# SpectacularAI/HybVIO

Hardware: NVIDIA H100
Metric: stereo frames/sec (752x480, 150 tracks) (higher is better)
Workload: dtype u8/s16 fixed-point + f32 (pyramid, LK), f64 (EKF)

## Files before the change

hybvio_b200/csrc/ekf.cuh:

```cuda
#pragma once
#include <cuda_runtime.h>

#define EKF_POS 0
#define EKF_VEL 3
#define EKF_ORI 6
#define EKF_BGA 10
#define EKF_BAA 13
#define EKF_BAT 16
#define EKF_SFT 19
#define EKF_CAM 20
#define EKF_INER 20
#define EKF_POSE 7
#define EKF_MAP_POINT 3
#define EKF_Q_ACC 0
#define EKF_Q_GYRO 3
#define EKF_Q_BGA_DRIFT 6
#define EKF_Q_BAA_DRIFT 9
#define EKF_Q_DIM 12

#define EKF_NT 512
#define EKF_SMALL_MAXN 8
#define EKF_SMALL_MAXL 32

struct EkfBufs {
    double* m;
    double* P;
    double* P2;
    double* work;
    double* cwork;
    double* Hs;
    double* Q;
    double* dydx;
    double* res;
    int N;
    int trail;
    int mapDim;
};

#define EKF_MODE_CHECK 0
#define EKF_MODE_UPDATE 1
#define EKF_MODE_CHECK_UPDATE 2

#define EKF_OP_DENSE 0
#define EKF_OP_ZUPT 1
#define EKF_OP_ZRUPT 2
#define EKF_OP_PSEUDO_VELOCITY 3
#define EKF_OP_POSITION 4
#define EKF_OP_ZERO_HEIGHT 5
#define EKF_OP_ORIENTATION 6
#define EKF_OP_AUGMENT 7

struct EkfUpdateArgs {
    EkfBufs b;
    const double* H;
    const double* f;
    const double* y;
    double ysmall[EKF_SMALL_MAXN];
    int n, l;
    int op;
    int mode;
    double Rdiag;
    double noiseScale;
    double rmseThr;
    double chi2Thr;
    int skipChi2;
    int normalizeAll;
    int symmetrize;
    int dropIdx;
    double augNoisePos, augNoiseOri;
    double defaultSpeed;
    int useGlobalWork;
    int symFirst;
    double* sig;
    double sigSeq;
    const int* gateI; int gateIExpect;
    const double* gateD; double gateDExpect;
    const int* counter; int counterMax;
    int* bump;
    double* slot;
    int lateH;
    int rowChunk;
    double* specP; double* specM;
    double Rdiag2;
};

__device__ __forceinline__ void ekf_report(const EkfUpdateArgs& a, double st, double chi2, double flag)
{
    a.b.res[0] = st; a.b.res[1] = chi2; a.b.res[2] = flag;
    if (a.slot) { a.slot[0] = st; a.slot[1] = chi2; a.slot[2] = flag; }
    if (a.sig) {
        a.sig[0] = st; a.sig[1] = chi2; a.sig[2] = flag;
        __threadfence_system();
        ((volatile double*)a.sig)[3] = a.sigSeq;
    }
}

#define EKF_MAX_BATCH 24
#define EKF_RES_STRIDE 32
struct EkfCheckItem {
    const double* H; const double* f; const double* y;
    int n, l;
    double Rdiag, chi2Thr, rmseThr;
    int skipChi2, pad;
};
struct EkfCheckBatch { int count; int pad; EkfCheckItem it[EKF_MAX_BATCH]; };

#define EKF_MAX_PREDICT 16
struct EkfPredictSample {
    double dt;
    double xg[3], xa[3];
    double baaDecay, bgaDecay;
    double qBaa, qBga;
    int normAfter, pad;
};
struct EkfPredictArgs {
    EkfBufs b;
    double gravity;
    double* meanOut;
    int count;
    EkfPredictSample s[EKF_MAX_PREDICT];
};

#define EKF_EW_SYMMETRIZE 1
#define EKF_EW_UNAUGMENT 2
#define EKF_EW_NORMALIZE 3
#define EKF_EW_TRANSLATE 4
#define EKF_EW_TRANSFORM 5
#define EKF_EW_INSERT_MAP_POINT 6
#define EKF_EW_LOCK_BIASES 7
#define EKF_EW_CONDITION_LAST_POSE 8
#define EKF_EW_INIT_ORIENTATION 9
struct EkfEwArgs {
    EkfBufs b;
    int op;
    int ival0;
    double dval[8];
};

cudaError_t ekf_launch_update(const EkfUpdateArgs& a, cudaStream_t s);
bool ekf_cluster2_fits(int n, int l, int N, bool joseph);
int ekf_cluster2_chunk_rows(int n, int l, int N);
cudaError_t ekf_launch_update_cluster2(const EkfUpdateArgs& a, cudaStream_t s);
cudaError_t ekf_launch_check_batch2(const EkfUpdateArgs& a, const EkfCheckBatch& b, cudaStream_t s, const EkfUpdateArgs* aug = nullptr);
cudaError_t ekf_launch_group_cluster2(const EkfUpdateArgs* hArgs, const EkfUpdateArgs* dArgs, int count, cudaStream_t s);
cudaError_t ekf_launch_group_predict(const EkfPredictArgs* hArgs, const EkfPredictArgs* dArgs, int count, cudaStream_t s);
struct TmArgs;
cudaError_t ekf_launch_predict(const EkfPredictArgs& a, cudaStream_t s);
cudaError_t ekf_launch_elementwise(const EkfEwArgs& a, cudaStream_t s);
```

hybvio_b200/csrc/ekf_cluster2.cu:

```cuda
#include <cooperative_groups.h>
#include "hv_device_once.cuh"
#include <math.h>
#include <stdlib.h>
namespace cg = cooperative_groups;

#ifdef HV_EKF_TIMING
#define EK2_PHASE(i) do { if (c == 0 && tid == 0) { unsigned long long t_; asm volatile("mov.u64 %0, %%globaltimer;" : "=l"(t_)); a.b.res[8 + (i)] = (double)t_; } } while (0)
#endif
#include "ekf_cluster2.cuh"

__global__ void __launch_bounds__(EK2_NT) ekf_update_cluster2_kernel(EkfUpdateArgs a)
{
    extern __shared__ __align__(16) double ek2_sm[];
    ek2_body<false>(a, ek2_sm, cg::this_cluster());
}

__global__ void __launch_bounds__(EK2_NT) ekf_update_cluster2_chunked_kernel(EkfUpdateArgs a)
{
    extern __shared__ __align__(16) double ek2_sm[];
    ek2_body<true>(a, ek2_sm, cg::this_cluster());
}

__global__ void __launch_bounds__(EK2_NT) ekf_check_batch_cluster2_kernel(EkfUpdateArgs a, EkfCheckBatch b, EkfUpdateArgs aug)
{
    extern __shared__ __align__(16) double ek2_sm[];
    cg::cluster_group cluster = cg::this_cluster();
    const int inst = blockIdx.x / EK2_C;
    if (inst >= b.count) a = aug;
    else {
        const EkfCheckItem& it = b.it[inst];
        a.H = it.H; a.f = it.f; a.y = it.y; a.n = it.n; a.l = it.l;
        a.Rdiag = it.Rdiag; a.chi2Thr = it.chi2Thr; a.rmseThr = it.rmseThr; a.skipChi2 = it.skipChi2;
        if (a.sig) a.sig += 4 * inst;
        if (a.slot) a.slot += 4 * inst;
    }
    a.b.res += (size_t)EKF_RES_STRIDE * inst;
    a.b.cwork += (size_t)inst * 10 * a.b.N * a.b.N;
    ek2_body<false>(a, ek2_sm, cluster);
}

__global__ void __launch_bounds__(EK2_NT) ekf_group_cluster2_kernel(const EkfUpdateArgs* __restrict__ args)
{
    extern __shared__ __align__(16) double ek2_sm[];
    ek2_group_body(args, blockIdx.x / EK2_C, ek2_sm, cg::this_cluster());
}

#define EK2_STATIC_SMEM (sizeof(double) * (2 + EK2_LINV_DOUBLES + 2 + EK2_MAXN) + 256)
#define EK2_SMEM_LIMIT (227 * 1024)

bool ekf_cluster2_fits(int n, int l, int N, bool joseph)
{
    return N <= EK2_MAXN && ek2_smem_bytes(n, l, N, joseph) + EK2_STATIC_SMEM <= EK2_SMEM_LIMIT;
}

int ekf_cluster2_chunk_rows(int n, int l, int N)
{
    if (N > EK2_MAXN) return 0;
    for (int h = n; h >= 1 && h >= (n < EK2_MIN_CHUNK ? n : EK2_MIN_CHUNK); h--)
        if (ek2_smem_bytes_chunked(h, n, l, N) + EK2_STATIC_SMEM <= EK2_SMEM_LIMIT) return h;
    return 0;
}

template <class K, class... Args>
static cudaError_t ek2_launch(K kernel, int nclusters, size_t smem, cudaStream_t s, Args... args)
{
    cudaLaunchConfig_t cfg = {};
    cfg.gridDim = dim3(EK2_C * nclusters); cfg.blockDim = dim3(EK2_NT); cfg.dynamicSmemBytes = smem; cfg.stream = s;
    cudaLaunchAttribute at[2];
    at[0].id = cudaLaunchAttributeClusterDimension; at[0].val.clusterDim.x = EK2_C; at[0].val.clusterDim.y = 1; at[0].val.clusterDim.z = 1;
    static const bool pdl = getenv("HV_EKF_NO_PDL") == nullptr;
    at[1].id = cudaLaunchAttributeProgrammaticStreamSerialization; at[1].val.programmaticStreamSerializationAllowed = 1;
    cfg.attrs = at; cfg.numAttrs = pdl ? 2 : 1;
    return cudaLaunchKernelEx(&cfg, kernel, args...);
}

template <class K>
static cudaError_t ek2_prepare(K kernel)
{
    return cudaFuncSetAttribute(kernel, cudaFuncAttributeMaxDynamicSharedMemorySize, (int)(EK2_SMEM_LIMIT - EK2_STATIC_SMEM));
}

cudaError_t ekf_launch_update_cluster2(const EkfUpdateArgs& a, cudaStream_t s)
{
    static bool seen[64], seenChunked[64];
    if (a.rowChunk > 0) {
        if (hv_first_use_on_device(seenChunked)) { cudaError_t e = ek2_prepare(ekf_update_cluster2_chunked_kernel); if (e != cudaSuccess) return e; }
        const size_t smem = ek2_smem_bytes_chunked(a.rowChunk < a.n ? a.rowChunk : a.n, a.n, a.l, a.b.N);
        return ek2_launch(ekf_update_cluster2_chunked_kernel, 1, smem, s, a);
    }
    if (hv_first_use_on_device(seen)) { cudaError_t e = ek2_prepare(ekf_update_cluster2_kernel); if (e != cudaSuccess) return e; }
    const size_t smem = ek2_smem_bytes(a.n, a.l, a.b.N, a.op == EKF_OP_AUGMENT);
    return ek2_launch(ekf_update_cluster2_kernel, 1, smem, s, a);
}

cudaError_t ekf_launch_check_batch2(const EkfUpdateArgs& a, const EkfCheckBatch& b, cudaStream_t s, const EkfUpdateArgs* aug)
{
    static bool seen[64];
    if (hv_first_use_on_device(seen)) { cudaError_t e = ek2_prepare(ekf_check_batch_cluster2_kernel); if (e != cudaSuccess) return e; }
    size_t smem = 0;
    for (int i = 0; i < b.count; i++) { const size_t v = ek2_smem_bytes(b.it[i].n, b.it[i].l, a.b.N, false); if (v > smem) smem = v; }
    if (aug) { const size_t v = ek2_smem_bytes(aug->n, aug->l, a.b.N, true); if (v > smem) smem = v; }
    return ek2_launch(ekf_check_batch_cluster2_kernel, b.count + (aug ? 1 : 0), smem, s, a, b, aug ? *aug : a);
}

cudaError_t ekf_launch_group_cluster2(const EkfUpdateArgs* hArgs, const EkfUpdateArgs* dArgs, int count, cudaStream_t s)
{
    static bool seen[64];
    if (hv_first_use_on_device(seen)) { cudaError_t e = ek2_prepare(ekf_group_cluster2_kernel); if (e != cudaSuccess) return e; }
    size_t smem = 0;
    for (int i = 0; i < count; i++) { const size_t v = ek2_smem_bytes(hArgs[i].n, hArgs[i].l, hArgs[i].b.N, hArgs[i].op == EKF_OP_AUGMENT); if (v > smem) smem = v; }
    return ek2_launch(ekf_group_cluster2_kernel, count, smem, s, dArgs);
}
```

hybvio_b200/csrc/ekf_cluster2.cuh:

```cuda
#pragma once
#include "ekf.cuh"
#include "hv_dmma.cuh"

#define EK2_NT 512
#define EK2_C 8
#define EK2_MAXN 768
#ifndef EK2_PHASE
#define EK2_PHASE(i) do { } while (0)
#endif
#ifndef EK2_ELIM_MARK
#define EK2_ELIM_MARK(i) do { } while (0)
#define EK2_ELIM_DECL
#endif

struct Ek2Geom { int B, X, W, T, PB, RS, EXTRA, SYM, oneStage, LD; };
__host__ __device__ inline int ek2_pad4mod16(int w) { return w + ((20 - (w & 15)) & 15); }
__host__ __device__ inline Ek2Geom ek2_geom(int n, int l, int N, bool joseph)
{
    Ek2Geom g;
    g.B = (N + EK2_C - 1) / EK2_C;
    g.LD = N + (((20 - (N & 15)) & 15) ? ((20 - (N & 15)) & 15) : 16);
    g.X = n * (l > g.LD ? l : g.LD);
    g.W = ek2_pad4mod16(n + g.B + 1 + (joseph ? n : 0));
    g.T = (n * g.W + 1) & ~1;
    g.PB = g.LD * g.B;
    const int MTn = (n + 7) >> 3;
    const int E = (64 * (MTn * (MTn + 1) / 2) + EK2_C - 1) / EK2_C;
    g.oneStage = n * n <= 1024 ? 1 : 0;
    g.RS = g.oneStage ? n * n : E;
    g.EXTRA = joseph ? N * EKF_POSE + 2 * 21 * g.LD + N * g.B : 0;
    g.SYM = n <= 8 ? N * g.B : 0;
    return g;
}
__host__ __device__ inline size_t ek2_smem_bytes(int n, int l, int N, bool joseph)
{
    const Ek2Geom g = ek2_geom(n, l, N, joseph);
    return ((size_t)g.X + g.T + g.PB + g.RS + g.EXTRA + g.SYM) * sizeof(double);
}
#define EK2_MIN_CHUNK 8
__host__ __device__ inline Ek2Geom ek2_geom_chunked(int h, int n, int l, int N)
{
    Ek2Geom g = ek2_geom(h, l, N, false);
    g.SYM = 0;
    g.EXTRA = (N + n + 1) & ~1;
    return g;
}
__host__ __device__ inline size_t ek2_smem_bytes_chunked(int h, int n, int l, int N)
{
    const Ek2Geom g = ek2_geom_chunked(h, n, l, N);
    return ((size_t)g.X + g.T + g.PB + g.RS + g.EXTRA) * sizeof(double);
}

__device__ __forceinline__ void ek2_copy8(double* __restrict__ dst, const double* __restrict__ src, int count, int tid)
{
    for (int base = 0; base < count; base += 8 * EK2_NT) {
        double r[8];
#pragma unroll
        for (int u = 0; u < 8; u++) { const int i = base + u * EK2_NT + tid; r[u] = i < count ? src[i] : 0.0; }
#pragma unroll
        for (int u = 0; u < 8; u++) { const int i = base + u * EK2_NT + tid; if (i < count) dst[i] = r[u]; }
    }
}
__device__ __forceinline__ void ek2_normalize_quat(double* q)
{
    const double z = (q[0] * q[0] + q[2] * q[2]) + (q[1] * q[1] + q[3] * q[3]);
    if (z > 0.0) { const double nrm = sqrt(z); q[0] /= nrm; q[1] /= nrm; q[2] /= nrm; q[3] /= nrm; }
}
__device__ __forceinline__ int ek2_aug_src(int i, int drop)
{
    if (i < EKF_CAM) return i;
    if (i < EKF_CAM + EKF_POSE) return -1;
    if (i < EKF_CAM + (drop + 1) * EKF_POSE) return i - EKF_POSE;
    return i;
}
__device__ __forceinline__ int ek2_special_col(int c) { return c < 3 ? EKF_POS + c : c < 7 ? EKF_ORI + c - 3 : EKF_CAM + c - 7; }

#define EK2_NI 4
__host__ __device__ inline void ek2_upper_tile(int tu, int& mt, int& nt)
{
    nt = (int)((sqrtf(8.0f * (float)tu + 1.0f) - 1.0f) * 0.5f);
    while ((nt + 1) * (nt + 2) / 2 <= tu) nt++;
    while (nt * (nt + 1) / 2 > tu) nt--;
    mt = tu - nt * (nt + 1) / 2;
}
template <int NI, bool UPPER, class FCI, class FST>
__device__ __forceinline__ void ek2_dmma_chunk(int M, int Nn, int K, int MT, int base, int stride, int lane, const double* A, int sAm, int sAk,
                                               const double* B, int sBk, int sBn, FCI cinit, FST store)
{
    const int g8 = lane >> 2, t4 = lane & 3;
    const int KF = K >> 2, tail = K & 3;
    const int dA = 4 * sAk, dB = 4 * sBk;
    double c0[NI], c1[NI];
    int row[NI], col[NI];
    const double* pa[NI]; const double* pb[NI];
#pragma unroll
    for (int q = 0; q < NI; q++) {
        const int tl = base + q * stride;
        int mt, nt;
        if (UPPER) ek2_upper_tile(tl, mt, nt); else { mt = tl % MT; nt = tl / MT; }
        row[q] = mt * 8 + g8; col[q] = nt * 8 + 2 * t4;
        const int rowc = min(row[q], M - 1), colbc = min(nt * 8 + g8, Nn - 1);
        pa[q] = A + (size_t)rowc * sAm + (size_t)t4 * sAk;
        pb[q] = B + (size_t)t4 * sBk + (size_t)colbc * sBn;
        c0[q] = cinit(rowc, min(col[q], Nn - 1)); c1[q] = cinit(rowc, min(col[q] + 1, Nn - 1));
    }
    int kt = 0;
    for (; kt + 2 <= KF; kt += 2) {
        double a0[NI], b0[NI], a1[NI], b1[NI];
#pragma unroll
        for (int q = 0; q < NI; q++) { a0[q] = pa[q][0]; b0[q] = pb[q][0]; a1[q] = pa[q][dA]; b1[q] = pb[q][dB]; pa[q] += 2 * dA; pb[q] += 2 * dB; }
#pragma unroll
        for (int q = 0; q < NI; q++) hv_dmma(c0[q], c1[q], a0[q], b0[q]);
#pragma unroll
        for (int q = 0; q < NI; q++) hv_dmma(c0[q], c1[q], a1[q], b1[q]);
    }
    if (kt < KF) {
        double a0[NI], b0[NI];
#pragma unroll
        for (int q = 0; q < NI; q++) { a0[q] = pa[q][0]; b0[q] = pb[q][0]; pa[q] += dA; pb[q] += dB; }
#pragma unroll
        for (int q = 0; q < NI; q++) hv_dmma(c0[q], c1[q], a0[q], b0[q]);
    }
    if (tail) {
        const bool kv = t4 < tail;
        double a0[NI], b0[NI];
#pragma unroll
        for (int q = 0; q < NI; q++) {
            const double xa = kv ? pa[q][0] : pa[q][-(ptrdiff_t)t4 * sAk];
            a0[q] = kv ? xa : 0.0;
            b0[q] = kv ? pb[q][0] : pb[q][-(ptrdiff_t)t4 * sBk];
        }
#pragma unroll
        for (int q = 0; q < NI; q++) hv_dmma(c0[q], c1[q], a0[q], b0[q]);
    }
    __syncwarp();
#pragma unroll
    for (int q = 0; q < NI; q++)
        if (row[q] < M && col[q] < Nn) store(row[q], col[q], c0[q], c1[q]);
}

template <bool UPPER = false, class FCI, class FST>
__device__ __forceinline__ void ek2_dmma_gemm(int M, int Nn, int K, int wrp, int lane, const double* A, int sAm, int sAk,
                                              const double* B, int sBk, int sBn, FCI cinit, FST store)
{
    const int MT = (M + 7) >> 3, NT = (Nn + 7) >> 3, tiles = UPPER ? MT * (MT + 1) / 2 : MT * NT;
    const int nwarps = EK2_NT / 32;
    if (M <= 0 || Nn <= 0) return;
    for (int base = wrp; base < tiles; base += nwarps * EK2_NI) {
        const int cnt = min(EK2_NI, (tiles - base + nwarps - 1) / nwarps);
        switch (cnt) {
            case 1: ek2_dmma_chunk<1, UPPER>(M, Nn, K, MT, base, nwarps, lane, A, sAm, sAk, B, sBk, sBn, cinit, store); break;
            case 2: ek2_dmma_chunk<2, UPPER>(M, Nn, K, MT, base, nwarps, lane, A, sAm, sAk, B, sBk, sBn, cinit, store); break;
            case 3: ek2_dmma_chunk<3, UPPER>(M, Nn, K, MT, base, nwarps, lane, A, sAm, sAk, B, sBk, sBn, cinit, store); break;
            default: ek2_dmma_chunk<4, UPPER>(M, Nn, K, MT, base, nwarps, lane, A, sAm, sAk, B, sBk, sBn, cinit, store); break;
        }
    }
}

#ifdef EK2_ELIM_OVERRIDE
#include EK2_ELIM_OVERRIDE
#else
#define EK2_LINV_DOUBLES 128
#define EK2_EB 8
__device__ __forceinline__ double ek2_rcp(double x)
{
#ifdef HV_EMU
    return 1.0 / x;
#else
    double r;
    asm("rcp.approx.ftz.f64 %0, %1;" : "=d"(r) : "d"(x));
    r = fma(fma(-x, r, 1.0), r, r);
    r = fma(fma(-x, r, 1.0), r, r);
    return r;
#endif
}

__device__ __forceinline__ void ek2_diag_factor(const double* T, int W, int r0, int nb, int lane, double* linv, volatile int* s_bad)
{
    double v[8];
    const int cidx = lane & 7;
#pragma unroll
    for (int i = 0; i < 8; i++) {
        const double t = T[(size_t)(r0 + min(i, nb - 1)) * W + r0 + min(cidx, nb - 1)];
        double x = (i == cidx) ? 1.0 : 0.0;
        if (lane < 8 && i < nb && cidx < nb) x = t;
        if (lane >= 16) x = 0.0;
        v[i] = x;
    }
    bool ok = true;
#pragma unroll
    for (int k = 0; k < 8; k++) {
        const double akk = __shfl_sync(0xffffffffu, v[k], k);
        double raw[8];
#pragma unroll
        for (int i = k + 1; i < 8; i++) raw[i] = __shfl_sync(0xffffffffu, v[k], i);
        if (!(akk > 0.0)) ok = false;
        const double r = rsqrt(akk);
        const double u = v[k] * r;
        v[k] = u;
#pragma unroll
        for (int i = k + 1; i < 8; i++) v[i] = fma(-(raw[i] * r), u, v[i]);
    }
    if (lane >= 8 && lane < 16) {
#pragma unroll
        for (int i = 0; i < 8; i++) linv[i * 8 + (lane - 8)] = v[i];
    }
    if (!ok && lane == 0) *s_bad = 1;
}

__device__ __forceinline__ bool ek2_block_eliminate(double* T, int W, int n, int ncols, int wrp, int lane, double* s_linv, volatile int* s_bad)
{
    const int g8 = lane >> 2, t4 = lane & 3;
    const int nwarps = EK2_NT / 32;
    const int MT = (n + 7) >> 3, CT = (ncols + 7) >> 3;
    EK2_ELIM_DECL
    if (wrp == 0) {
        if (lane == 0) *s_bad = 0;
        __syncwarp();
        ek2_diag_factor(T, W, 0, min(8, n), lane, s_linv, s_bad);
    }
    __syncthreads();
    for (int j = 0; j < MT; j++) {
        if (*s_bad) return false;
        const int r0 = 8 * j, nb = min(8, n - r0);
        const double* linv = s_linv + (j & 1) * 64;
        EK2_ELIM_MARK(0);
        for (int ct = j + wrp; ct < CT; ct += nwarps) {
            double c0 = 0.0, c1 = 0.0;
            const int colbc = min(8 * ct + g8, ncols - 1);
            double bf[2];
#pragma unroll
            for (int kt = 0; kt < 2; kt++) {
                const int k = kt * 4 + t4;
                const double x = T[(size_t)(r0 + min(k, nb - 1)) * W + colbc];
                bf[kt] = k < nb ? x : 0.0;
            }
#pragma unroll
            for (int kt = 0; kt < 2; kt++) hv_dmma(c0, c1, linv[g8 * 8 + kt * 4 + t4], bf[kt]);
            const int col = 8 * ct + 2 * t4;
            __syncwarp();
            if (g8 < nb) { if (col < ncols) T[(size_t)(r0 + g8) * W + col] = c0; if (col + 1 < ncols) T[(size_t)(r0 + g8) * W + col + 1] = c1; }
        }
        EK2_ELIM_MARK(1);
        __syncthreads();
        EK2_ELIM_MARK(2);
        if (j + 1 < MT) {
            const int first = j + 1;
            int total = 0;
            for (int mt = first; mt < MT; mt++) total += CT - mt;
            const bool ahead = wrp == 0;
            const int nwork = nwarps - nwarps / 4, widx = wrp - wrp / 4 - 1;
            const bool worker = (wrp & 3) != 0;
            const int rest = total - 1;
            int lo = ahead ? 0 : worker ? 1 + (int)(((long long)rest * widx) / nwork) : 0;
            const int hi = ahead ? 1 : worker ? 1 + (int)(((long long)rest * (widx + 1)) / nwork) : 0;
            const double* rowk0 = T + (size_t)(r0 + min(t4, nb - 1)) * W;
            const double* rowk1 = T + (size_t)(r0 + min(4 + t4, nb - 1)) * W;
            const bool k0v = t4 < nb, k1v = 4 + t4 < nb;
            if (ahead) {
                const int cb = 8 * first, am = min(cb + g8, ncols - 1);
                const double x0 = rowk0[am], x1 = rowk1[am];
                const int rowi = cb + g8, coli = cb + 2 * t4;
                double* crow = T + (size_t)min(rowi, n - 1) * W;
                double c0 = crow[min(coli, ncols - 1)], c1 = crow[min(coli + 1, ncols - 1)];
                hv_dmma(c0, c1, k0v ? -x0 : 0.0, x0);
                hv_dmma(c0, c1, k1v ? -x1 : 0.0, x1);
                __syncwarp();
                if (rowi < n) { if (coli < ncols) crow[coli] = c0; if (coli + 1 < ncols) crow[coli + 1] = c1; }
            } else if (worker) {
                int mt = first, nt, idx = min(lo, total - 1);
                while (idx >= CT - mt) { idx -= CT - mt; mt++; }
                nt = mt + idx;
                int curMt = -1;
                double a0 = 0.0, a1 = 0.0;
                for (; lo < hi; lo++) {
                    if (mt != curMt) {
                        const int am = min(8 * mt + g8, ncols - 1);
                        const double x0 = rowk0[am], x1 = rowk1[am];
                        a0 = k0v ? -x0 : 0.0; a1 = k1v ? -x1 : 0.0;
                        curMt = mt;
                    }
                    const int rowi = 8 * mt + g8, coli = 8 * nt + 2 * t4, bn = min(8 * nt + g8, ncols - 1);
                    double* crow = T + (size_t)min(rowi, n - 1) * W;
                    double c0 = crow[min(coli, ncols - 1)], c1 = crow[min(coli + 1, ncols - 1)];
                    const double b0 = rowk0[bn], b1 = rowk1[bn];
                    hv_dmma(c0, c1, a0, b0);
                    hv_dmma(c0, c1, a1, b1);
                    __syncwarp();
                    if (rowi < n) { if (coli < ncols) crow[coli] = c0; if (coli + 1 < ncols) crow[coli + 1] = c1; }
                    if (++nt == CT) { mt++; nt = mt; }
                }
            }
            EK2_ELIM_MARK(3);
            if (ahead) {
                __syncwarp();
                ek2_diag_factor(T, W, 8 * first, min(8, n - 8 * first), lane, s_linv + (first & 1) * 64, s_bad);
            }
            EK2_ELIM_MARK(4);
            __syncthreads();
            EK2_ELIM_MARK(5);
        }
    }
    return !*s_bad;
}

#endif

__device__ __forceinline__ void ek2_pdl_launch_dependents()
{
#ifndef HV_EMU
    asm volatile("griddepcontrol.launch_dependents;" ::: "memory");
#endif
}
__device__ __forceinline__ void ek2_pdl_wait()
{
#ifndef HV_EMU
    asm volatile("griddepcontrol.wait;" ::: "memory");
#endif
}

__device__ __forceinline__ void ek2_bar_init(unsigned long long* bar, int count)
{
#ifdef HV_EMU
    *bar = 0; (void)count;
#else
    asm volatile("mbarrier.init.shared::cta.b64 [%0], %1;" :: "r"((unsigned)__cvta_generic_to_shared(bar)), "r"(count) : "memory");
    asm volatile("fence.proxy.async.shared::cta;" ::: "memory");
#endif
}
__device__ __forceinline__ void ek2_bar_expect(unsigned long long* bar, unsigned bytes)
{
#ifdef HV_EMU
    (void)bar; (void)bytes;
#else
    if (bytes) asm volatile("mbarrier.arrive.expect_tx.shared::cta.b64 _, [%0], %1;" :: "r"((unsigned)__cvta_generic_to_shared(bar)), "r"(bytes) : "memory");
    else asm volatile("mbarrier.arrive.shared::cta.b64 _, [%0];" :: "r"((unsigned)__cvta_generic_to_shared(bar)) : "memory");
#endif
}
__device__ __forceinline__ void ek2_bar_wait(unsigned long long* bar, unsigned phase)
{
#ifdef HV_EMU
    (void)bar; (void)phase;
#else
    unsigned done;
    do {
        asm volatile("{\n\t.reg .pred p;\n\tmbarrier.try_wait.parity.shared::cta.b64 p, [%1], %2;\n\tselp.b32 %0, 1, 0, p;\n\t}"
                     : "=r"(done) : "r"((unsigned)__cvta_generic_to_shared(bar)), "r"(phase) : "memory");
    } while (!done);
#endif
}
__device__ __forceinline__ void ek2_bulk_g2s(double* dst, const double* src, unsigned bytes, unsigned long long* bar)
{
#ifdef HV_EMU
    if ((((size_t)dst) | ((size_t)src) | bytes) & 15) { fprintf(stderr, "emu: misaligned bulk copy (global -> shared)\n"); abort(); }
    memcpy(dst, src, bytes); (void)bar;
#else
    asm volatile("cp.async.bulk.shared::cluster.global.mbarrier::complete_tx::bytes [%0], [%1], %2, [%3];"
                 :: "r"((unsigned)__cvta_generic_to_shared(dst)), "l"(src), "r"(bytes), "r"((unsigned)__cvta_generic_to_shared(bar)) : "memory");
#endif
}
__device__ __forceinline__ void ek2_bulk_s2g(double* dst, const double* src, unsigned bytes)
{
#ifdef HV_EMU
    if ((((size_t)dst) | ((size_t)src) | bytes) & 15) { fprintf(stderr, "emu: misaligned bulk copy (shared -> global)\n"); abort(); }
    memcpy(dst, src, bytes);
#else
    asm volatile("cp.async.bulk.global.shared::cta.bulk_group [%0], [%1], %2;" :: "l"(dst), "r"((unsigned)__cvta_generic_to_shared(src)), "r"(bytes) : "memory");
#endif
}
__device__ __forceinline__ void ek2_bulk_store_done()
{
#ifndef HV_EMU
    asm volatile("cp.async.bulk.commit_group;" ::: "memory");
    asm volatile("cp.async.bulk.wait_group 0;" ::: "memory");
#endif
}
__device__ __forceinline__ void ek2_fence_async_smem()
{
#ifndef HV_EMU
    asm volatile("fence.proxy.async.shared::cta;" ::: "memory");
#endif
}
__device__ __forceinline__ void ek2_fence_async_all()
{
#ifndef HV_EMU
    asm volatile("fence.proxy.async;" ::: "memory");
#endif
}

template <bool CHUNKS = true, class Cluster>
__device__ __forceinline__ void ek2_body(EkfUpdateArgs& a, double* sm, Cluster cluster)
{
    __shared__ double s_scalar[2];
    __shared__ double s_linv[EK2_LINV_DOUBLES];
    __shared__ int s_bad;
    __shared__ __align__(16) double s_m[EK2_MAXN];
    __shared__ __align__(8) unsigned long long s_bar[4];
    const int c = (int)cluster.block_rank(), C = (int)cluster.num_blocks();
    const int tid = threadIdx.x, lane = tid & 31, wrp = tid >> 5, nwarps = EK2_NT / 32;
    const int N = a.b.N, n = a.n, l = a.l;
    const bool joseph = a.op == EKF_OP_AUGMENT;
    const bool chunked = CHUNKS && a.rowChunk > 0;
    const int hc = chunked ? min(a.rowChunk, n) : n;
    const Ek2Geom g = chunked ? ek2_geom_chunked(hc, n, l, N) : ek2_geom(n, l, N, joseph);
    double* X = sm;
    double* T = X + g.X;
    double* PB = T + g.T;
    double* RS = PB + g.PB;
    double* EX = RS + g.RS;
    double* SYMB = EX + g.EXTRA;
    double* const DM = EX;
    double* const VF = EX + N;
    const int W = g.W, B = g.B, LD = g.LD;
    const int J0 = c * B, Bc = max(0, min(B, N - J0));
    const int vcol = n + B;
    const bool oneStage = g.oneStage != 0;
    double* const Sred = a.b.cwork + (size_t)N * N;
    double* const Spart = a.b.cwork + (size_t)2 * N * N;
    double* const P = a.b.P;

    EK2_PHASE(0);
    ek2_pdl_launch_dependents();
    const bool bulk = (N & 1) == 0 && ((((size_t)P) | ((size_t)a.b.m) | ((size_t)a.b.cwork) | ((size_t)a.specP) | ((size_t)a.specM) | ((size_t)sm)) & 15) == 0;
    const bool bulkH = bulk && !chunked && a.op == EKF_OP_DENSE && ((n * l) & 1) == 0 && (((size_t)a.H) & 15) == 0;
    if (tid == 0) { ek2_bar_init(&s_bar[0], 2); ek2_bar_init(&s_bar[1], 1); ek2_bar_init(&s_bar[2], 1); ek2_bar_init(&s_bar[3], 1); }
    if (bulk) __syncthreads();
    const bool lateH = a.lateH != 0 && a.op == EKF_OP_DENSE;
    if (a.op == EKF_OP_DENSE) {
        if (!lateH && !chunked) {
            if (bulkH) { if (tid == 0) { ek2_bar_expect(&s_bar[0], (unsigned)(n * l * 8)); ek2_bulk_g2s(X, a.H, (unsigned)(n * l * 8), &s_bar[0]); } }
            else ek2_copy8(X, a.H, n * l, tid);
        }
    } else for (int i = tid; i < n * l; i += EK2_NT) X[i] = 0.0;
    ek2_pdl_wait();
    if (a.gateI || a.gateD || a.counter) {
        bool run = true;
        if (a.gateI && *(volatile const int*)a.gateI != a.gateIExpect) run = false;
        if (a.gateD && *(volatile const double*)a.gateD != a.gateDExpect) run = false;
        if (a.counter && *(volatile const int*)a.counter >= a.counterMax) run = false;
        if (!run) {
            if (bulk) {
                const int arrived = (bulkH && !lateH) ? 1 : 0;
                if (tid == 0) for (int q = arrived; q < 2; q++) ek2_bar_expect(&s_bar[0], 0);
                ek2_bar_wait(&s_bar[0], 0);
            }
            if (c == 0 && tid == 0) ekf_report(a, 1.0, 0.0, 0.0);
            return;
        }
    }
    if (lateH && !chunked) {
        if (bulkH) { if (tid == 0) { ek2_bar_expect(&s_bar[0], (unsigned)(n * l * 8)); ek2_bulk_g2s(X, a.H, (unsigned)(n * l * 8), &s_bar[0]); } }
        else ek2_copy8(X, a.H, n * l, tid);
    }
    if (bulk && !bulkH && tid == 0) ek2_bar_expect(&s_bar[0], 0);
    if (joseph) {
        const int drop = a.dropIdx;
        for (int i = tid; i < N; i += EK2_NT) { const int s = ek2_aug_src(i, drop); s_m[i] = s < 0 ? 0.0 : a.b.m[s]; }
        for (int idx = tid; idx < N * Bc; idx += EK2_NT) {
            const int i = idx % N, j = J0 + idx / N;
            const int si = ek2_aug_src(i, drop), sj = ek2_aug_src(j, drop);
            double v = (si < 0 || sj < 0) ? 0.0 : P[si + (size_t)sj * N];
            if (a.symFirst && si >= 0 && sj >= 0 && si != sj) v = 0.5 * (v + P[sj + (size_t)si * N]);
            if (i == j && i >= EKF_CAM && i < EKF_CAM + EKF_POSE) v += (i - EKF_CAM) < 3 ? a.augNoisePos : a.augNoiseOri;
            PB[i + (size_t)(idx / N) * LD] = v;
        }
        if (bulk && tid == 0) ek2_bar_expect(&s_bar[0], 0);
    } else if (bulk) {
        if (wrp == 0) {
            if (lane == 0) ek2_bar_expect(&s_bar[0], (unsigned)((N * Bc + N) * 8));
            __syncwarp();
            for (int j = lane; j < Bc; j += 32) ek2_bulk_g2s(PB + (size_t)j * LD, P + (size_t)(J0 + j) * N, (unsigned)(N * 8), &s_bar[0]);
            if (lane == 31) ek2_bulk_g2s(s_m, a.b.m, (unsigned)(N * 8), &s_bar[0]);
        }
    } else {
        for (int i = tid; i < N; i += EK2_NT) s_m[i] = a.b.m[i];
        const double* src = P + (size_t)J0 * N;
        const int count = N * Bc;
        for (int base = 0; base < count; base += 8 * EK2_NT) {
            double r[8];
#pragma unroll
            for (int u = 0; u < 8; u++) { const int i = base + u * EK2_NT + tid; r[u] = i < count ? src[i] : 0.0; }
#pragma unroll
            for (int u = 0; u < 8; u++) { const int i = base + u * EK2_NT + tid; if (i < count) PB[(i % N) + (size_t)(i / N) * LD] = r[u]; }
        }
    }

    if (bulk) ek2_bar_wait(&s_bar[0], 0);
    double hspeed = 0.0;
    if (a.op == EKF_OP_DENSE) {
        __syncthreads();
    } else {
        __syncthreads();
        if (a.op == EKF_OP_PSEUDO_VELOCITY) {
            hspeed = sqrt(s_m[EKF_VEL] * s_m[EKF_VEL] + s_m[EKF_VEL + 1] * s_m[EKF_VEL + 1]);
            if (hspeed <= 1e-7) return;
        }
        if (tid == 0) {
            switch (a.op) {
                case EKF_OP_ZUPT: for (int i = 0; i < 3; i++) X[i + (EKF_VEL + i) * n] = 1.0; break;
                case EKF_OP_ZRUPT: for (int i = 0; i < 3; i++) X[i + (EKF_BGA + i) * n] = 1.0; break;
                case EKF_OP_PSEUDO_VELOCITY: for (int i = 0; i < 2; i++) X[(EKF_VEL + i) * n] = s_m[EKF_VEL + i] / hspeed; break;
                case EKF_OP_POSITION: for (int i = 0; i < 3; i++) X[i + (EKF_POS + i) * n] = 1.0; break;
                case EKF_OP_ZERO_HEIGHT: X[(EKF_POS + 2) * n] = 1.0; break;
                case EKF_OP_ORIENTATION: for (int i = 0; i < 4; i++) X[i + (EKF_ORI + i) * n] = 1.0; break;
                case EKF_OP_AUGMENT:
                    for (int i = 0; i < 3; i++) { X[i + (EKF_POS + i) * n] = 1.0; X[i + (EKF_CAM + i) * n] = -1.0; }
                    for (int i = 0; i < 4; i++) { X[3 + i + (EKF_ORI + i) * n] = 1.0; X[3 + i + (EKF_CAM + 3 + i) * n] = -1.0; }
                    break;
            }
        }
        __syncthreads();
    }
    const double* Hs = X;

    const double* Hf = chunked ? a.H : Hs;
    for (int i = tid; i < n; i += EK2_NT) {
        double v;
        if (a.op == EKF_OP_PSEUDO_VELOCITY) v = a.defaultSpeed - hspeed;
        else {
            const double yi = a.y ? a.y[i] : a.ysmall[i];
            double fi = 0.0;
            if (a.f) fi = a.f[i];
            else for (int k = 0; k < l; k++) fi += Hf[i + (size_t)k * n] * s_m[k];
            v = yi - fi;
        }
        if (chunked) VF[i] = v;
        else T[(size_t)i * W + vcol] = v;
    }
    if (joseph) for (int t = tid; t < n * n; t += EK2_NT) T[(size_t)(t / n) * W + vcol + 1 + (t % n)] = (t / n == t % n) ? 1.0 : 0.0;
    __syncthreads();

    const bool checking = a.mode != EKF_MODE_UPDATE;
    if (checking && a.rmseThr >= 0.0) {
        if (tid == 0) { double ss = 0.0; for (int i = 0; i < n; i++) { const double v = chunked ? VF[i] : T[(size_t)i * W + vcol]; ss += v * v; } s_scalar[0] = sqrt(ss / n); }
        __syncthreads();
        if (s_scalar[0] > a.rmseThr) { if (c == 0 && tid == 0) ekf_report(a, 2.0, 0.0, 0.0); return; }
    }
    if (checking && a.skipChi2 && a.mode == EKF_MODE_CHECK) {
        if (c == 0 && tid == 0) ekf_report(a, 0.0, 0.0, 0.0);
        return;
    }

    if (chunked) {
        for (int i = tid; i < N; i += EK2_NT) DM[i] = 0.0;
        __syncthreads();
    }

    const bool twoPass = chunked && a.Rdiag2 > 0.0 && a.mode == EKF_MODE_CHECK_UPDATE && !a.skipChi2;
    int pass = 0, r0 = 0;
    double Rk = a.Rdiag, chi2sum = 0.0;
    unsigned zph = 0, sph = 0;
    double* const Z = X;
    const int cm = (N - 1) / B;
    for (;;) {
        const int nr = chunked ? min(hc, n - r0) : n;
        const bool lastChunk = r0 + nr >= n;
        const bool decideOnly = chunked && checking && pass == 0 && (a.mode == EKF_MODE_CHECK || twoPass);
        const int vk = nr + B, cend = joseph ? vk + nr : vk;
        const int MTs = (nr + 7) >> 3, ETOT = 64 * (MTs * (MTs + 1) / 2);
        if (chunked) {
            if (pass > 0 || r0 > 0) cluster.sync();
            for (int t = tid; t < nr * l; t += EK2_NT) { const int i = t % nr, k = t / nr; X[t] = a.H[r0 + i + (size_t)k * n]; }
            __syncthreads();
            for (int i = tid; i < nr; i += EK2_NT) {
                double v = VF[r0 + i];
                for (int k = 0; k < l; k++) v -= X[i + (size_t)k * nr] * DM[k];
                T[(size_t)i * W + vk] = v;
            }
            __syncthreads();
        }

        EK2_PHASE(1);
        ek2_dmma_gemm(nr, Bc, l, wrp, lane, Hs, 1, nr, PB, 1, LD,
                      [](int, int) { return 0.0; },
                      [&](int i, int j, double v0, double v1) { T[(size_t)i * W + nr + j] = v0; if (j + 1 < Bc) T[(size_t)i * W + nr + j + 1] = v1; });
        __syncthreads();
        EK2_PHASE(2);
        {
            const int kc = max(0, min(Bc, l - J0));
            ek2_dmma_gemm<true>(nr, nr, kc, wrp, lane, T + nr, W, 1, Hs + (size_t)J0 * nr, nr, 1,
                          [](int, int) { return 0.0; },
                          [&](int i, int j, double v0, double v1) {
                              if (oneStage) { RS[i * nr + j] = v0; if (j + 1 < nr) RS[i * nr + j + 1] = v1; }
                              else {
                                  const int mt = i >> 3, nt = j >> 3;
                                  double* dst = Spart + (size_t)c * ETOT + 64 * (nt * (nt + 1) / 2 + mt) + 8 * (i & 7) + (j & 7);
                                  dst[0] = v0; dst[1] = v1;
                              }
                          });
        }
        EK2_PHASE(3);
        if (!oneStage && bulk) ek2_fence_async_all();
        cluster.sync();
        {
            auto entry = [&](int e, int& i, int& ip) { int mt, nt; ek2_upper_tile(e >> 6, mt, nt); i = 8 * mt + ((e >> 3) & 7); ip = 8 * nt + (e & 7); };
            if (oneStage) {
                for (int e = tid; e < ETOT; e += EK2_NT) {
                    int i, ip; entry(e, i, ip);
                    if (i < nr && ip < nr) {
                        double s = 0.0;
                        for (int r = 0; r < C; r++) s += cluster.map_shared_rank(RS, r)[i * nr + ip];
                        if (i == ip) s += Rk;
                        T[(size_t)i * W + ip] = s;
                    }
                }
                __syncthreads();
            } else if (bulk && ETOT >= 2048 && ETOT % (2 * C) == 0 && 2 * ETOT <= g.X) {
                const int E = ETOT / C, e0 = c * E;
                double* SL = X + ETOT;
                if (wrp == 0) {
                    if (lane == 0) ek2_bar_expect(&s_bar[2], (unsigned)(C * E * 8));
                    __syncwarp();
                    if (lane < C) ek2_bulk_g2s(SL + (size_t)lane * E, Spart + (size_t)lane * ETOT + e0, (unsigned)(E * 8), &s_bar[2]);
                }
                ek2_bar_wait(&s_bar[2], sph);
                __syncthreads();
                for (int q = tid; q < E; q += EK2_NT) {
                    const int e = e0 + q;
                    int i, ip; entry(e, i, ip);
                    double sacc = 0.0;
                    if (i < nr && ip < nr) {
                        for (int r = 0; r < C; r++) sacc += SL[(size_t)r * E + q];
                        if (i == ip) sacc += Rk;
                    }
                    Sred[e] = sacc;
                }
                ek2_fence_async_all();
                cluster.sync();
                if (tid == 0) { ek2_bar_expect(&s_bar[3], (unsigned)(ETOT * 8)); ek2_bulk_g2s(X, Sred, (unsigned)(ETOT * 8), &s_bar[3]); }
                ek2_bar_wait(&s_bar[3], sph);
                sph ^= 1;
                __syncthreads();
                for (int tu = wrp; tu < ETOT / 64; tu += nwarps) {
                    int mt, nt; ek2_upper_tile(tu, mt, nt);
#pragma unroll
                    for (int h = 0; h < 2; h++) {
                        const int q = lane + 32 * h, i = 8 * mt + (q >> 3), ip = 8 * nt + (q & 7);
                        if (i < nr && ip < nr) T[(size_t)i * W + ip] = X[64 * tu + q];
                    }
                }
                __syncthreads();
            } else {
                const int E = (ETOT + C - 1) / C, e0 = c * E, e1 = min(ETOT, e0 + E);
                for (int e = e0 + tid; e < e1; e += EK2_NT) {
                    int i, ip; entry(e, i, ip);
                    double s = 0.0;
                    if (i < nr && ip < nr) {
                        for (int r = 0; r < C; r++) s += Spart[(size_t)r * ETOT + e];
                        if (i == ip) s += Rk;
                    }
                    Sred[e] = s;
                }
                cluster.sync();
                for (int tu = wrp; tu < ETOT / 64; tu += nwarps) {
                    int mt, nt; ek2_upper_tile(tu, mt, nt);
#pragma unroll
                    for (int h = 0; h < 2; h++) {
                        const int q = lane + 32 * h, e = 64 * tu + q, i = 8 * mt + (q >> 3), ip = 8 * nt + (q & 7);
                        if (i < nr && ip < nr) T[(size_t)i * W + ip] = Sred[e];
                    }
                }
                __syncthreads();
            }
        }

        EK2_PHASE(4);
        bool decided = false;
        if (!chunked && a.Rdiag2 > 0.0 && a.mode == EKF_MODE_CHECK_UPDATE && a.op == EKF_OP_DENSE && !a.skipChi2) {
            const int W2 = min(ek2_pad4mod16(n + 1), max(l, LD));
            double* Xc = X;
            for (int e = tid; e < n * n; e += EK2_NT) Xc[(size_t)(e / n) * W2 + (e % n)] = T[(size_t)(e / n) * W + (e % n)];
            for (int i = tid; i < n; i += EK2_NT) Xc[(size_t)i * W2 + n] = T[(size_t)i * W + vcol];
            __syncthreads();
            for (int i = tid; i < n; i += EK2_NT) T[(size_t)i * W + i] += a.Rdiag2 - a.Rdiag;
            const bool bad2 = !ek2_block_eliminate(Xc, W2, n, n + 1, wrp, lane, s_linv, &s_bad);
            if (bad2) {
                if (c == 0 && tid == 0) ekf_report(a, 1.0, 0.0, 1.0);
                cluster.sync();
                return;
            }
            __syncthreads();
            if (wrp == 0) {
                double t = 0.0;
                for (int k = lane; k < n; k += 32) { const double z = Xc[(size_t)k * W2 + n]; t += z * z; }
#pragma unroll
                for (int o = 16; o > 0; o >>= 1) t += __shfl_sync(0xffffffffu, t, lane ^ o);
                if (lane == 0) s_scalar[1] = a.noiseScale * t;
            }
            __syncthreads();
            const double chi2c = s_scalar[1];
            const bool outlier = chi2c > a.chi2Thr;
            if (c == 0 && tid == 0) ekf_report(a, outlier ? 3.0 : 0.0, chi2c, 0.0);
            if (outlier) { cluster.sync(); return; }
            decided = true;
            __syncthreads();
        }
        const bool bad = !ek2_block_eliminate(T, W, nr, cend + 1, wrp, lane, s_linv, &s_bad);
        if (bad) {
            if (c == 0 && tid == 0) ekf_report(a, 1.0, 0.0, 1.0);
            if (a.specP) {
                for (int idx = tid; idx < N * Bc; idx += EK2_NT) a.specP[(size_t)J0 * N + idx] = P[(size_t)J0 * N + idx];
                if (c == 0) for (int i = tid; i < N; i += EK2_NT) a.specM[i] = a.b.m[i];
            }
            cluster.sync();
            return;
        }
        __syncthreads();
        EK2_PHASE(5);
        if (wrp == 0) {
            double t = 0.0;
            for (int k = lane; k < nr; k += 32) { const double z = T[(size_t)k * W + vk]; t += z * z; }
#pragma unroll
            for (int o = 16; o > 0; o >>= 1) t += __shfl_sync(0xffffffffu, t, lane ^ o);
            if (lane == 0) s_scalar[1] = a.noiseScale * t;
        }
        __syncthreads();
        const double chi2 = s_scalar[1];
        if (chunked) {
            chi2sum += chi2;
        } else if (decided) {
        } else if (checking) {
            const bool outlier = !a.skipChi2 && chi2 > a.chi2Thr;
            if (c == 0 && tid == 0) ekf_report(a, outlier ? 3.0 : 0.0, chi2, 0.0);
            if (outlier || a.mode == EKF_MODE_CHECK) { cluster.sync(); return; }
        } else if (c == 0 && tid == 0) ekf_report(a, 0.0, chi2, 0.0);

        if (!(lastChunk && decideOnly)) {
            EK2_PHASE(6);
            if ((size_t)nr * N >= 4096) {
                double* Zg = a.b.cwork;
                for (int t = tid; t < nr * Bc; t += EK2_NT) { const int k = t / Bc, jj = t - k * Bc; Zg[(size_t)k * N + J0 + jj] = T[(size_t)k * W + nr + jj]; }
                if (bulk) ek2_fence_async_all();
                cluster.sync();
                if (bulk) {
                    if (wrp == 0) {
                        if (lane == 0) ek2_bar_expect(&s_bar[1], (unsigned)(nr * N * 8));
                        __syncwarp();
                        for (int k = lane; k < nr; k += 32) ek2_bulk_g2s(Z + (size_t)k * LD, Zg + (size_t)k * N, (unsigned)(N * 8), &s_bar[1]);
                    }
                    ek2_bar_wait(&s_bar[1], zph);
                    zph ^= 1;
                } else
                for (int base = 0; base < nr * N; base += 8 * EK2_NT) {
                    double r[8];
#pragma unroll
                    for (int u = 0; u < 8; u++) { const int t = base + u * EK2_NT + tid; r[u] = t < nr * N ? Zg[t] : 0.0; }
#pragma unroll
                    for (int u = 0; u < 8; u++) { const int t = base + u * EK2_NT + tid; if (t < nr * N) Z[(size_t)(t / N) * LD + (t % N)] = r[u]; }
                }
            } else {
                cluster.sync();
                for (int t = tid; t < nr * N; t += EK2_NT) {
                    const int k = t / N, col = t - k * N, r = col / B;
                    Z[(size_t)k * LD + col] = cluster.map_shared_rank(T, r)[(size_t)k * W + nr + (col - r * B)];
                }
            }
            if (!chunked && c == cm) for (int k = tid; k < n; k += EK2_NT) Z[(size_t)k * LD + N] = T[(size_t)k * W + vcol];
            __syncthreads();
            EK2_PHASE(7);
            {
                const int own = !chunked && c == cm ? 1 : 0;
                ek2_dmma_gemm(N, Bc + own, nr, wrp, lane, Z, 1, LD, Z + J0, LD, 1,
                              [&](int i, int j) { return j < Bc ? -PB[i + (size_t)j * LD] : s_m[i]; },
                              [&](int i, int j, double v0, double v1) {
                                  if (j < Bc) PB[i + (size_t)j * LD] = -v0; else s_m[i] = v0;
                                  if (j + 1 < Bc) PB[i + (size_t)(j + 1) * LD] = -v1; else if (j + 1 == Bc && own) s_m[i] = v1;
                              });
            }
            if (chunked)
                for (int i = tid; i < N; i += EK2_NT) {
                    double s = DM[i];
                    for (int k = 0; k < nr; k++) s += Z[(size_t)k * LD + i] * T[(size_t)k * W + vk];
                    DM[i] = s;
                }
        }
        if (!chunked) break;
        if (!lastChunk) { r0 += nr; continue; }
        if (checking && pass == 0) {
            const bool outlier = !a.skipChi2 && chi2sum > a.chi2Thr;
            if (c == 0 && tid == 0) ekf_report(a, outlier ? 3.0 : 0.0, chi2sum, 0.0);
            if (outlier || a.mode == EKF_MODE_CHECK) { cluster.sync(); return; }
            if (twoPass) {
                const double* src = P + (size_t)J0 * N;
                for (int idx = tid; idx < N * Bc; idx += EK2_NT) PB[(idx % N) + (size_t)(idx / N) * LD] = src[idx];
                for (int i = tid; i < N; i += EK2_NT) DM[i] = 0.0;
                pass = 1; r0 = 0; chi2sum = 0.0; Rk = a.Rdiag2;
                continue;
            }
        } else if (!checking && c == 0 && tid == 0) ekf_report(a, 0.0, chi2sum, 0.0);
        break;
    }
    if (joseph) {
        double* Ks = EX;
        for (int t = tid; t < N * EKF_POSE; t += EK2_NT) {
            const int i = t % N, r = t / N;
            double s = 0.0;
            for (int k = 0; k < n; k++) s += Z[(size_t)k * LD + i] * T[(size_t)k * W + vcol + 1 + r];
            Ks[t] = s;
        }
    }
    if (bulk) ek2_fence_async_smem();
    __syncthreads();
    if (c == cm) {
        if (chunked) {
            for (int i = tid; i < N; i += EK2_NT) s_m[i] += DM[i];
            __syncthreads();
        }
        for (int q = tid; q < (a.normalizeAll ? a.b.trail + 1 : 1); q += EK2_NT)
            ek2_normalize_quat(q == 0 ? s_m + EKF_ORI : s_m + EKF_CAM + EKF_POSE * (q - 1) + 3);
        ek2_fence_async_smem();
        __syncthreads();
        double* const mDst = a.specM ? a.specM : a.b.m;
        if (bulk) { if (tid == 32) { ek2_bulk_s2g(mDst, s_m, (unsigned)(N * 8)); ek2_bulk_store_done(); } }
        else for (int i = tid; i < N; i += EK2_NT) mDst[i] = s_m[i];
    }
    EK2_PHASE(8);

    double* Pblk = PB;
    int ldb = LD;
    if (joseph) {
        double* Ks = EX;
        double* AS = Ks + (size_t)N * EKF_POSE;
        double* BS = AS + (size_t)21 * LD;
        double* P2 = BS + (size_t)21 * LD;
        EK2_PHASE(10);
        for (int t = tid; t < N * 21; t += EK2_NT) {
            const int j = t % N, cc = t / N;
            if (cc < 14) {
                const double kv = cc < 7 ? -Ks[j + cc * N] : Ks[j + (cc - 7) * N];
                BS[j + (size_t)cc * LD] = (j == ek2_special_col(cc) ? 1.0 : 0.0) + kv;
            } else {
                BS[j + (size_t)cc * LD] = a.Rdiag * Ks[j + (cc - 14) * N];
                AS[j + (size_t)cc * LD] = Ks[j + (cc - 14) * N];
            }
        }
        EK2_PHASE(11);
        cluster.sync();
        EK2_PHASE(12);
        for (int t = tid; t < N * 14; t += EK2_NT) {
            const int i = t % N, cc = t / N;
            const int col = ek2_special_col(cc), r = col / B;
            AS[i + (size_t)cc * LD] = cluster.map_shared_rank(PB, r)[i + (size_t)(col - r * B) * LD];
        }
        __syncthreads();
        EK2_PHASE(13);
        ek2_dmma_gemm(N, Bc, 21, wrp, lane, AS, 1, LD, BS + J0, LD, 1,
                      [&](int i, int jj) {
                          const int j = J0 + jj;
                          const bool jsp = j < 3 || (j >= EKF_ORI && j < EKF_ORI + 4) || (j >= EKF_CAM && j < EKF_CAM + EKF_POSE);
                          return jsp ? 0.0 : PB[i + (size_t)jj * LD];
                      },
                      [&](int i, int jj, double v0, double v1) { P2[i + (size_t)jj * N] = v0; if (jj + 1 < Bc) P2[i + (size_t)(jj + 1) * N] = v1; });
        Pblk = P2; ldb = N;
        EK2_PHASE(14);
    }
    double* const Pdst = a.specP ? a.specP : P;
    if (a.symmetrize) {
        if (joseph) __syncthreads();
        for (int idx = tid; idx < N * Bc; idx += EK2_NT) {
            const int jrow = idx % N, icol = idx / N, r = jrow / B;
            cluster.map_shared_rank(SYMB, r)[(J0 + icol) + (size_t)(jrow - r * B) * N] = Pblk[jrow + (size_t)icol * ldb];
        }
        cluster.sync();
        EK2_PHASE(15);
        for (int idx = tid; idx < N * Bc; idx += EK2_NT) {
            const int i = idx % N, jj = idx / N, j = J0 + jj;
            double v = Pblk[i + (size_t)jj * ldb];
            const double w = SYMB[idx];
            if (i != j) v = i > j ? 0.5 * (v + w) : 0.5 * (w + v);
            Pdst[i + (size_t)j * N] = v;
        }
    } else if (bulk) {
        if (wrp == 0) {
            for (int j = lane; j < Bc; j += 32) ek2_bulk_s2g(Pdst + (size_t)(J0 + j) * N, Pblk + (size_t)j * ldb, (unsigned)(N * 8));
            ek2_bulk_store_done();
        }
    } else {
        for (int idx = tid; idx < N * Bc; idx += EK2_NT) Pdst[(size_t)J0 * N + idx] = Pblk[(idx % N) + (size_t)(idx / N) * ldb];
    }
    EK2_PHASE(9);
    if (a.bump && c == 0 && tid == 0) *a.bump = *a.bump + 1;
    cluster.sync();
}

template <class Cluster>
__device__ __forceinline__ void ek2_group_body(const EkfUpdateArgs* __restrict__ args, int inst, double* sm, Cluster cluster)
{
    EkfUpdateArgs a = args[inst];
    ek2_body<false>(a, sm, cluster);
}
```

Before: 4151.

## Run small EKF chi2 checks on single CTAs instead of full clusters

Batched chi2 check items that are small enough (l <= N, bounded n*l*l, fitting shared memory) are now packed one per CTA, eight per cluster, and computed by a new single-CTA routine. That routine computes H P H^T + R with DMMA GEMMs over column blocks of P and then does a block elimination. Each such check previously occupied an 8-CTA cluster with cross-CTA synchronisation; the aim is to cut that cluster overhead and free SMs. The cost is that each check now runs serially within one CTA, and items are mapped to blocks by a linear scan of the batch.

```diff
diff --git a/hybvio_b200/csrc/ekf.cuh b/hybvio_b200/csrc/ekf.cuh
--- a/hybvio_b200/csrc/ekf.cuh
+++ b/hybvio_b200/csrc/ekf.cuh
@@ -101,9 +101,10 @@
     const double* H; const double* f; const double* y;
     int n, l;
     double Rdiag, chi2Thr, rmseThr;
-    int skipChi2, pad;
+    int skipChi2;
+    int compact;
 };
-struct EkfCheckBatch { int count; int pad; EkfCheckItem it[EKF_MAX_BATCH]; };
+struct EkfCheckBatch { int count; int compact; EkfCheckItem it[EKF_MAX_BATCH]; };
 
 #define EKF_MAX_PREDICT 16
 struct EkfPredictSample {
diff --git a/hybvio_b200/csrc/ekf_cluster2.cu b/hybvio_b200/csrc/ekf_cluster2.cu
--- a/hybvio_b200/csrc/ekf_cluster2.cu
+++ b/hybvio_b200/csrc/ekf_cluster2.cu
@@ -21,11 +21,21 @@
     ek2_body<true>(a, ek2_sm, cg::this_cluster());
 }
 
+__device__ __forceinline__ int ek2_batch_item(const EkfCheckBatch& b, int compact, int j)
+{
+    for (int i = 0; i < b.count; i++)
+        if (b.it[i].compact == compact && j-- == 0) return i;
+    return compact ? -1 : b.count;
+}
+
 __global__ void __launch_bounds__(EK2_NT) ekf_check_batch_cluster2_kernel(EkfUpdateArgs a, EkfCheckBatch b, EkfUpdateArgs aug)
 {
     extern __shared__ __align__(16) double ek2_sm[];
     cg::cluster_group cluster = cg::this_cluster();
-    const int inst = blockIdx.x / EK2_C;
+    const int k = blockIdx.x / EK2_C, compactClusters = (b.compact + EK2_C - 1) / EK2_C;
+    const bool compact = k < compactClusters;
+    const int inst = compact ? ek2_batch_item(b, 1, k * EK2_C + (int)cluster.block_rank()) : ek2_batch_item(b, 0, k - compactClusters);
+    if (inst < 0) return;
     if (inst >= b.count) a = aug;
     else {
         const EkfCheckItem& it = b.it[inst];
@@ -35,9 +45,11 @@
         if (a.slot) a.slot += 4 * inst;
     }
     a.b.res += (size_t)EKF_RES_STRIDE * inst;
+    if (compact) { ek2_check_cta(a, ek2_sm); return; }
     a.b.cwork += (size_t)inst * 10 * a.b.N * a.b.N;
     ek2_body<false>(a, ek2_sm, cluster);
 }
+static_assert(2 * sizeof(EkfUpdateArgs) + sizeof(EkfCheckBatch) <= 4096, "ekf_check_batch_cluster2_kernel: arguments beyond 4 KB of parameter space");
 
 __global__ void __launch_bounds__(EK2_NT) ekf_group_cluster2_kernel(const EkfUpdateArgs* __restrict__ args)
 {
@@ -93,14 +105,31 @@
     return ek2_launch(ekf_update_cluster2_kernel, 1, smem, s, a);
 }
 
-cudaError_t ekf_launch_check_batch2(const EkfUpdateArgs& a, const EkfCheckBatch& b, cudaStream_t s, const EkfUpdateArgs* aug)
+#define EK2_CTA_CHECK_MAX (1 << 20)
+static bool ekf_check_on_one_cta(int n, int l, int N)
+{
+    return l <= N && (long long)n * l * l <= EK2_CTA_CHECK_MAX && ek2_check_cta_smem_bytes(n, l, N) + EK2_STATIC_SMEM <= EK2_SMEM_LIMIT;
+}
+
+cudaError_t ekf_launch_check_batch2(const EkfUpdateArgs& a, const EkfCheckBatch& b0, cudaStream_t s, const EkfUpdateArgs* aug)
 {
     static bool seen[64];
     if (hv_first_use_on_device(seen)) { cudaError_t e = ek2_prepare(ekf_check_batch_cluster2_kernel); if (e != cudaSuccess) return e; }
+    EkfCheckBatch b = b0;
+    b.compact = 0;
+    int clusters = aug ? 1 : 0;
     size_t smem = 0;
-    for (int i = 0; i < b.count; i++) { const size_t v = ek2_smem_bytes(b.it[i].n, b.it[i].l, a.b.N, false); if (v > smem) smem = v; }
+    for (int i = 0; i < b.count; i++) {
+        EkfCheckItem& it = b.it[i];
+        it.compact = ekf_check_on_one_cta(it.n, it.l, a.b.N) ? 1 : 0;
+        const size_t v = it.compact ? ek2_check_cta_smem_bytes(it.n, it.l, a.b.N) : ek2_smem_bytes(it.n, it.l, a.b.N, false);
+        if (v > smem) smem = v;
+        b.compact += it.compact;
+        clusters += 1 - it.compact;
+    }
+    clusters += (b.compact + EK2_C - 1) / EK2_C;
     if (aug) { const size_t v = ek2_smem_bytes(aug->n, aug->l, a.b.N, true); if (v > smem) smem = v; }
-    return ek2_launch(ekf_check_batch_cluster2_kernel, b.count + (aug ? 1 : 0), smem, s, a, b, aug ? *aug : a);
+    return ek2_launch(ekf_check_batch_cluster2_kernel, clusters, smem, s, a, b, aug ? *aug : a);
 }
 
 cudaError_t ekf_launch_group_cluster2(const EkfUpdateArgs* hArgs, const EkfUpdateArgs* dArgs, int count, cudaStream_t s)
diff --git a/hybvio_b200/csrc/ekf_cluster2.cuh b/hybvio_b200/csrc/ekf_cluster2.cuh
--- a/hybvio_b200/csrc/ekf_cluster2.cuh
+++ b/hybvio_b200/csrc/ekf_cluster2.cuh
@@ -883,6 +883,103 @@
     cluster.sync();
 }
 
+struct Ek2CheckGeom { int B, W, LDP, X, T; };
+#define EK2_CTA_SCRATCH (EK2_LINV_DOUBLES + 4)
+__host__ __device__ inline Ek2CheckGeom ek2_check_geom(int n, int l, int N)
+{
+    Ek2CheckGeom g;
+    g.B = (N + EK2_C - 1) / EK2_C;
+    g.W = ek2_pad4mod16(n + 1 + g.B);
+    g.LDP = ek2_pad4mod16(l);
+    g.X = (n * l + 1) & ~1;
+    g.T = (n * g.W + 1) & ~1;
+    return g;
+}
+__host__ __device__ inline size_t ek2_check_cta_smem_bytes(int n, int l, int N)
+{
+    const Ek2CheckGeom g = ek2_check_geom(n, l, N);
+    return ((size_t)EK2_CTA_SCRATCH + g.X + g.T + (size_t)g.LDP * g.B) * sizeof(double);
+}
+
+#ifdef HV_EMU
+#define EK2_NOINLINE inline
+#else
+#define EK2_NOINLINE __noinline__
+#endif
+__device__ EK2_NOINLINE void ek2_check_cta(const EkfUpdateArgs& a, double* sm)
+{
+    const int tid = threadIdx.x, lane = tid & 31, wrp = tid >> 5;
+    const int N = a.b.N, n = a.n, l = a.l;
+    const Ek2CheckGeom g = ek2_check_geom(n, l, N);
+    const int W = g.W, B = g.B, LDP = g.LDP;
+    double* const s_linv = sm;
+    double* const s_scalar = sm + EK2_LINV_DOUBLES;
+    volatile int* const s_bad = (volatile int*)(sm + EK2_LINV_DOUBLES + 2);
+    double* const Hs = sm + EK2_CTA_SCRATCH;
+    double* const T = Hs + g.X;
+    double* const PB = T + g.T;
+    ek2_pdl_launch_dependents();
+    if (!a.lateH) ek2_copy8(Hs, a.H, n * l, tid);
+    ek2_pdl_wait();
+    if (a.lateH) ek2_copy8(Hs, a.H, n * l, tid);
+    __syncthreads();
+    for (int i = tid; i < n; i += EK2_NT) {
+        const double yi = a.y ? a.y[i] : a.ysmall[i];
+        double fi = 0.0;
+        if (a.f) fi = a.f[i];
+        else for (int k = 0; k < l; k++) fi += Hs[i + (size_t)k * n] * a.b.m[k];
+        T[(size_t)i * W + n] = yi - fi;
+    }
+    for (int e = tid; e < n * n; e += EK2_NT) T[(size_t)(e / n) * W + (e % n)] = 0.0;
+    __syncthreads();
+    if (a.rmseThr >= 0.0) {
+        if (tid == 0) { double ss = 0.0; for (int i = 0; i < n; i++) { const double v = T[(size_t)i * W + n]; ss += v * v; } s_scalar[0] = sqrt(ss / n); }
+        __syncthreads();
+        if (s_scalar[0] > a.rmseThr) { if (tid == 0) ekf_report(a, 2.0, 0.0, 0.0); return; }
+    }
+    if (a.skipChi2) { if (tid == 0) ekf_report(a, 0.0, 0.0, 0.0); return; }
+
+    for (int c = 0; c < EK2_C; c++) {
+        const int J0 = c * B, kc = min(B, l - J0);
+        if (kc <= 0) break;
+        const double* src = a.b.P + (size_t)J0 * N;
+        const int count = l * kc;
+        for (int base = 0; base < count; base += 8 * EK2_NT) {
+            double r[8];
+#pragma unroll
+            for (int u = 0; u < 8; u++) { const int t = base + u * EK2_NT + tid, j = t / l; r[u] = t < count ? src[(t - j * l) + (size_t)j * N] : 0.0; }
+#pragma unroll
+            for (int u = 0; u < 8; u++) { const int t = base + u * EK2_NT + tid, j = t / l; if (t < count) PB[(t - j * l) + (size_t)j * LDP] = r[u]; }
+        }
+        __syncthreads();
+        ek2_dmma_gemm(n, kc, l, wrp, lane, Hs, 1, n, PB, 1, LDP,
+                      [](int, int) { return 0.0; },
+                      [&](int i, int j, double v0, double v1) { T[(size_t)i * W + n + 1 + j] = v0; if (j + 1 < kc) T[(size_t)i * W + n + 2 + j] = v1; });
+        __syncthreads();
+        ek2_dmma_gemm<true>(n, n, kc, wrp, lane, T + n + 1, W, 1, Hs + (size_t)J0 * n, n, 1,
+                            [](int, int) { return 0.0; },
+                            [&](int i, int j, double v0, double v1) { T[(size_t)i * W + j] += v0; if (j + 1 < n) T[(size_t)i * W + j + 1] += v1; });
+        __syncthreads();
+    }
+    for (int i = tid; i < n; i += EK2_NT) T[(size_t)i * W + i] += a.Rdiag;
+    __syncthreads();
+    if (!ek2_block_eliminate(T, W, n, n + 1, wrp, lane, s_linv, s_bad)) {
+        if (tid == 0) ekf_report(a, 1.0, 0.0, 1.0);
+        return;
+    }
+    __syncthreads();
+    if (wrp == 0) {
+        double t = 0.0;
+        for (int k = lane; k < n; k += 32) { const double z = T[(size_t)k * W + n]; t += z * z; }
+#pragma unroll
+        for (int o = 16; o > 0; o >>= 1) t += __shfl_sync(0xffffffffu, t, lane ^ o);
+        if (lane == 0) s_scalar[1] = a.noiseScale * t;
+    }
+    __syncthreads();
+    const double chi2 = s_scalar[1];
+    if (tid == 0) ekf_report(a, chi2 > a.chi2Thr ? 3.0 : 0.0, chi2, 0.0);
+}
+
 template <class Cluster>
 __device__ __forceinline__ void ek2_group_body(const EkfUpdateArgs* __restrict__ args, int inst, double* sm, Cluster cluster)
 {
```

After: 4511, median of 6. 8.7% higher.
